# JMIsham/flink

Hardware: AMD Instinct MI355X
Metric: records/sec keyed windowed aggregation at 1/2/4/8 GPUs; % of HBM roofline (higher is better)
Workload: dtype int64

## Files before the change

flink_amd/csrc/fw_device.hip:

```cpp
#include <hip/hip_runtime.h>
#include <hip/hip_ext.h>

#include <algorithm>
#include <rocprim/device/device_radix_sort.hpp>

#include "../../include/flink_window.h"
#include "fw_internal.h"

namespace {

constexpr int64_t LMAX = INT64_MAX;
constexpr int64_t LMIN = INT64_MIN;
typedef long long i64x2 __attribute__((ext_vector_type(2)));
typedef uint32_t u32x4 __attribute__((ext_vector_type(4)));

#include "fw_jmath.h"
__device__ __forceinline__ uint64_t fmix64_inv(uint64_t x) {
  x ^= x >> 33;
  x *= 0x9cb4b2f8129337dbull;
  x ^= x >> 33;
  x *= 0x4f74430c22a54005ull;
  x ^= x >> 33;
  return x;
}
// ... 334 lines not shown
    }
  }
  return -1;
}
template <bool OWN = false>
__device__ __forceinline__ int32_t region_claim(const Region& r, uint64_t h, uint32_t word) {
  for (uint32_t i = 0; i <= r.mask; i++) {
    const uint32_t s = ((uint32_t)h + i) & r.mask;
    if ((OWN ? ld_state_wg(r.state + s) : ld_state(r.state + s)) != SLOT_EMPTY) continue;
    if ((OWN ? cas_state_wg(r.state + s, SLOT_EMPTY, word) : atomicCAS(r.state + s, SLOT_EMPTY, word)) == SLOT_EMPTY)
      return (int32_t)s;
  }
  return -1;
}


constexpr uint32_t TAINT_BUSY = 0x80000000u;
constexpr int TAINT_MAX_PROBES = 64;
__device__ __forceinline__ bool taint_insert(const DevCfg& c, int64_t key) {
  uint32_t s = taint_slot0(c, key);
  for (int probes = 0; probes < TAINT_MAX_PROBES;) {
    const uint32_t cur = __hip_atomic_load(&c.taint_state[s], __ATOMIC_RELAXED, __HIP_MEMORY_SCOPE_AGENT);
    __atomic_signal_fence(__ATOMIC_ACQUIRE);
    if (cur == c.taint_epoch) {
      if (__hip_atomic_load(&c.taint_key[s], __ATOMIC_RELAXED, __HIP_MEMORY_SCOPE_AGENT) == (uint64_t)key) return true;
      s = (s + 1) & c.taint_mask;
      probes++;
      continue;
    }
    if (cur == (c.taint_epoch | TAINT_BUSY)) continue;
    if (atomicCAS(&c.taint_state[s], cur, c.taint_epoch | TAINT_BUSY) == cur) {
      __hip_atomic_store(&c.taint_key[s], (uint64_t)key, __ATOMIC_RELAXED, __HIP_MEMORY_SCOPE_AGENT);
      asm volatile("s_waitcnt vmcnt(0)" ::: "memory");
      __hip_atomic_store(&c.taint_state[s], c.taint_epoch, __ATOMIC_RELAXED, __HIP_MEMORY_SCOPE_AGENT);
      return true;
    }
  }
  return false;
}
__global__ __launch_bounds__(256) void k_taint(DevCfg c, int64_t wm, const int64_t* __restrict__ key,
                                               const int64_t* __restrict__ ts, int64_t n, Status* st) {
  int any = 0;
  for (int64_t i = (int64_t)blockIdx.x * blockDim.x + threadIdx.x; i < n; i += (int64_t)gridDim.x * blockDim.x) {
    if (!session_ordered(c, wm, ts[i])) continue;
    any = max(any, taint_insert(c, key[i]) ? 1 : 2);
  }
  if (any) atomicMax(&st->taint_any, any);
}

__device__ __forceinline__ int64_t rec_index(int64_t b, int j, int e) {
  return b + 2 * ((int64_t)j * blockDim.x + threadIdx.x) + e;
}
template <int NP, bool VAL>
__device__ __forceinline__ void load_records(const DevCfg& c, const int64_t* __restrict__ key, const int64_t* __restrict__ ts,
                                             const int64_t* __restrict__ val, const int32_t* __restrict__ kh, int64_t b,
                                             int64_t end, int64_t (&k)[2 * NP], int64_t (&t)[2 * NP], int64_t (&v)[2 * NP],
                                             int32_t (&h)[2 * NP]) {
  const bool hashed = c.key_kind == FW_KEY_HASHED;
#pragma unroll
  for (int j = 0; j < NP; j++) {
    const int64_t i = rec_index(b, j, 0);
    if (c.vec_in && i + 1 < end) {
      const i64x2 kk = *reinterpret_cast<const i64x2*>(key + i);
      const i64x2 tt = *reinterpret_cast<const i64x2*>(ts + i);
      k[2 * j] = kk.x, k[2 * j + 1] = kk.y;
      t[2 * j] = tt.x, t[2 * j + 1] = tt.y;
      if (VAL) {
        const i64x2 vv = *reinterpret_cast<const i64x2*>(val + i);
        v[2 * j] = vv.x, v[2 * j + 1] = vv.y;
      }
      if (hashed) {
        const int2 hh = *reinterpret_cast<const int2*>(kh + i);
        h[2 * j] = hh.x, h[2 * j + 1] = hh.y;
      }
    } else {
#pragma unroll
      for (int e = 0; e < 2; e++) {
        const bool in = i + e < end;
        k[2 * j + e] = in ? key[i + e] : 0;
        t[2 * j + e] = in ? ts[i + e] : 0;
        if (VAL) v[2 * j + e] = in ? val[i + e] : 0;
        if (hashed) h[2 * j + e] = in ? kh[i + e] : 0;
      }
    }
  }
}
__device__ __forceinline__ int32_t tile_of_block(int32_t T) {
  const int32_t b = blockIdx.x;
  if (!FW_XCD_TILES) return b;
  const int32_t per = T >> 3, rem = T & 7, g = b & 7;
  return g * per + min(g, rem) + (b >> 3);
}

enum { M_GEN = 0, M_TUMB = 1, M_PANE = 2 };
template <int MODE>
__device__ __forceinline__ void specialize(DevCfg& c) {
  if constexpr (MODE == M_TUMB) {
    c.assigner = FW_TUMBLING;
    c.panes = 0;
    c.wpr = 1;
    c.key_kind = FW_KEY_LONG;
  } else if constexpr (MODE == M_PANE) {
    c.assigner = FW_SLIDING;
    c.panes = 1;
    c.key_kind = FW_KEY_LONG;
  }
}
__host__ __forceinline__ int stream_mode(const DevCfg& c) {
  if (c.key_kind != FW_KEY_LONG) return M_GEN;
  if (c.assigner == FW_TUMBLING) return M_TUMB;
  return c.panes ? M_PANE : M_GEN;
}

enum { RSV_OVER = 0, RSV_KG = 1, RSV_TS = 2, RSV_LATE = 4 };

template <int MODE>
__global__ __launch_bounds__(FW_TILE_THREADS) void k_classify_hist(DevCfg c, int64_t wm, const int64_t* __restrict__ key,
                                                                   const int64_t* __restrict__ ts,
                                                                   const int32_t* __restrict__ kh, int64_t n, int32_t T,
                                                                   uint32_t* __restrict__ hist, Status* st,
                                                                   const uint32_t* __restrict__ rsv) {
  specialize<MODE>(c);
  if (rsv && !rsv[c.P + RSV_OVER]) {
    if (blockIdx.x == 0 && threadIdx.x == 0) {
      if (rsv[c.P + RSV_KG]) atomicAdd(&st->kg_errors, (int)rsv[c.P + RSV_KG]);
      if (rsv[c.P + RSV_TS]) atomicAdd(&st->ts_errors, (int)rsv[c.P + RSV_TS]);
      const unsigned long long late = *reinterpret_cast<const unsigned long long*>(rsv + c.P + RSV_LATE);
      if (late) atomicAdd(&st->late_dropped, late);
    }
    return;
  }
  if (rsv && blockIdx.x == 0 && threadIdx.x == 0) {
    if (rsv[c.P + FW_RSV_NARROW])
      atomicAdd(&st->narrow_misses, 1);
    else
      atomicAdd(&st->rsv_fallbacks, 1);
  }
  extern __shared__ uint32_t lh[];
  for (int i = threadIdx.x; i <= c.P; i += blockDim.x) lh[i] = 0;
  __syncthreads();
  const int32_t tile = blockIdx.x;
  const int64_t base = (int64_t)tile * FW_TILE;
  const int64_t end = min(n, base + (int64_t)FW_TILE);
  int bad_kg = 0, bad_ts = 0, wide = 0;
  unsigned slow = 0;
  const int taint = c.assigner == FW_SESSION ? st->taint_any : 0;
  for (int64_t b = base; b < end; b += (int64_t)blockDim.x * FW_RPT) {
    int64_t k[FW_RPT], t[FW_RPT], v[FW_RPT];
    int32_t h[FW_RPT];
    load_records<FW_RPT / 2, false>(c, key, ts, nullptr, kh, b, end, k, t, v, h);
#pragma unroll
    for (int j = 0; j < FW_RPT; j++) {
      const int64_t i = rec_index(b, j >> 1, j & 1);
      if (i >= end) continue;
      const int32_t p = partition_of(c, k[j], c.key_kind == FW_KEY_HASHED ? h[j] : key_hash_of(c.key_kind, k[j], kh, i));
      if (p < 0) {
        bad_kg++;
        continue;
      }
      int64_t last = 0;
      int nw = 0;
      const int cls = classify(c, wm, t[j], &last, &nw, k[j], taint);
      if (cls == CLS_NORMAL) {
        atomicAdd(&lh[p], 1u);
        if (c.compact && compact_delta(c, last) < 0) wide = 1;
      } else if (cls == CLS_SLOW)
        slow++;
      else if (cls == CLS_BADTS)
        bad_ts++;
    }
  }
  if (slow) atomicAdd(&lh[c.P], slow);
  __syncthreads();
  for (int i = threadIdx.x; i <= c.P; i += blockDim.x) hist[(int64_t)i * T + tile] = lh[i];
  if (threadIdx.x == 0) hist[(int64_t)(c.P + 1) * T + tile] = lh[c.P];
  if (bad_kg) atomicAdd(&st->kg_errors, bad_kg);
  if (bad_ts) atomicAdd(&st->ts_errors, bad_ts);
  if (wide) atomicOr(c.wide, 1);
}

constexpr int SCAN_T = 1024, SCAN_E = 4, SCAN_B = SCAN_T * SCAN_E;

__device__ __forceinline__ uint32_t block_excl_scan(uint32_t v, uint32_t* sw, uint32_t* total) {
  const int lane = __lane_id(), wid = threadIdx.x >> 6;
  uint32_t x = v;
#pragma unroll
  for (int o = 1; o < 64; o <<= 1) {
    uint32_t y = __shfl_up(x, o, 64);
    if (lane >= o) x += y;
  }
  if (lane == 63) sw[wid] = x;
  __syncthreads();
  if (threadIdx.x == 0) {
    uint32_t run = 0;
    const int nw = blockDim.x >> 6;
    for (int w = 0; w < nw; w++) {
      uint32_t t = sw[w];
      sw[w] = run;
      run += t;
    }
    sw[nw] = run;
  }
  __syncthreads();
  *total = sw[blockDim.x >> 6];
  uint32_t r = sw[wid] + x - v;
  __syncthreads();
  return r;
}

__global__ __launch_bounds__(SCAN_T) void k_scan_blocks(uint32_t* data, int64_t m, uint32_t* sums, const uint32_t* gate) {
  if (gate && !*gate) return;
  __shared__ uint32_t sw[SCAN_T / 64 + 1];
  const int64_t base = (int64_t)blockIdx.x * SCAN_B + (int64_t)threadIdx.x * SCAN_E;
  uint32_t v[SCAN_E];
  uint32_t local = 0;
#pragma unroll
  for (int e = 0; e < SCAN_E; e++) {
    v[e] = base + e < m ? data[base + e] : 0u;
    local += v[e];
  }
  uint32_t total;
  uint32_t off = block_excl_scan(local, sw, &total);
#pragma unroll
  for (int e = 0; e < SCAN_E; e++) {
    if (base + e < m) data[base + e] = off;
    off += v[e];
  }
  if (threadIdx.x == 0) sums[blockIdx.x] = total;
}
__global__ __launch_bounds__(SCAN_T) void k_scan_top(uint32_t* sums, int64_t nb, const uint32_t* gate) {
  if (gate && !*gate) return;
  __shared__ uint32_t sw[SCAN_T / 64 + 1];
  uint32_t carry = 0;
  for (int64_t b0 = 0; b0 < nb; b0 += SCAN_T) {
    const int64_t i = b0 + threadIdx.x;
    uint32_t v = i < nb ? sums[i] : 0u, total;
    uint32_t off = block_excl_scan(v, sw, &total);
    if (i < nb) sums[i] = off + carry;
    carry += total;
  }
}
__global__ __launch_bounds__(SCAN_T) void k_scan_add(uint32_t* data, int64_t m, const uint32_t* sums, const uint32_t* gate) {
  if (gate && !*gate) return;
  const uint32_t add = sums[blockIdx.x];
  const int64_t base = (int64_t)blockIdx.x * SCAN_B;
  for (int e = threadIdx.x; e < SCAN_B; e += SCAN_T)
    if (base + e < m) data[base + e] += add;
}

__global__ __launch_bounds__(SCAN_T) void k_scan_gated(uint32_t* data, int64_t m, const uint32_t* gate) {
  if (!*gate) return;
  __shared__ uint32_t sw[SCAN_T / 64 + 1];
  uint32_t carry = 0;
  for (int64_t b0 = 0; b0 < m; b0 += SCAN_B) {
    const int64_t base = b0 + (int64_t)threadIdx.x * SCAN_E;
    uint32_t v[SCAN_E];
    uint32_t local = 0;
#pragma unroll
    for (int e = 0; e < SCAN_E; e++) {
      v[e] = base + e < m ? data[base + e] : 0u;
      local += v[e];
    }
    uint32_t total;
    uint32_t off = block_excl_scan(local, sw, &total) + carry;
#pragma unroll
    for (int e = 0; e < SCAN_E; e++) {
      if (base + e < m) data[base + e] = off;
      off += v[e];
    }
    carry += total;
    __syncthreads();
  }
}

__device__ __forceinline__ uint32_t dpp_swap1(uint32_t x) {
  return (uint32_t)__builtin_amdgcn_mov_dpp((int)x, 0xB1, 0xF, 0xF, false);
}
__device__ __forceinline__ int64_t dpp_swap1(int64_t x) {
  const uint32_t lo = dpp_swap1((uint32_t)(uint64_t)x), hi = dpp_swap1((uint32_t)((uint64_t)x >> 32));
  return (int64_t)(((uint64_t)hi << 32) | lo);
}
__device__ __forceinline__ void store_pair(PRec* part, bool valid, uint32_t pos, i64x2 a, i64x2 b) {
  const bool odd = __lane_id() & 1;
  const i64x2 send = odd ? a : b;
  const i64x2 recv = {dpp_swap1((int64_t)send.x), dpp_swap1((int64_t)send.y)};
  const uint32_t ppos = dpp_swap1(pos);
  const bool pval = dpp_swap1((uint32_t)valid) != 0;
  if (odd ? pval : valid) reinterpret_cast<i64x2*>(part + (odd ? ppos : pos))[odd] = odd ? recv : a;
  if (odd ? valid : pval) reinterpret_cast<i64x2*>(part + (odd ? pos : ppos))[odd] = odd ? b : recv;
}
// ... 7 lines not shown
  __syncthreads();
  const int64_t tbase = (int64_t)tile * FW_TILE;
  const int64_t tend = min(n, tbase + (int64_t)FW_TILE);
  unsigned long long late = 0;
  const int taint = c.assigner == FW_SESSION ? st->taint_any : 0;
  const bool cmp = c.compact && !*c.wide;
  for (int64_t b = tbase; b < tend; b += (int64_t)blockDim.x * FW_RPT) {
    int64_t k[FW_RPT], t[FW_RPT], v[FW_RPT];
    int32_t hh[FW_RPT];
    load_records<FW_RPT / 2, true>(c, key, ts, val, kh, b, tend, k, t, v, hh);
#pragma unroll
    for (int j = 0; j < FW_RPT; j++) {
      const int64_t i = rec_index(b, j >> 1, j & 1);
      bool norm = false;
      uint32_t pos = 0;
      int64_t last = 0;
      int nwin = 0;
      if (i < tend) {
        const int32_t h = c.key_kind == FW_KEY_HASHED ? hh[j] : key_hash_of(c.key_kind, k[j], kh, i);
        const int32_t p = partition_of(c, k[j], h);
        if (p >= 0) {
          const int cls = classify(c, wm, t[j], &last, &nwin, k[j], taint);
          if (cls == CLS_NORMAL) {
            pos = atomicAdd(&base[p], 1u);
            norm = true;
          } else if (cls == CLS_LATE) {
            if (c.side_output)
              side_one(side, st, k[j], t[j], v[j]);
            else
              late++;
          }
        }
      }
      if (c.diag & (DIAG_SCATTER_NO_STORE | DIAG_SCATTER_LINEAR | DIAG_SCATTER_SINGLE | DIAG_SCATTER_HALF |
                    DIAG_SCATTER_NT)) {
        if (c.diag & DIAG_SCATTER_NO_STORE) {
          asm volatile("" ::"v"(pos), "v"(k[j]), "v"(last), "v"(v[j]));
          continue;
        }
        if (c.diag & DIAG_SCATTER_LINEAR) pos = (uint32_t)i;
        if ((c.diag & DIAG_SCATTER_HALF) && norm) {
          i64x2* dst = reinterpret_cast<i64x2*>(part) + pos;
          if (c.diag & DIAG_SCATTER_NT)
            __builtin_nontemporal_store(i64x2{k[j] ^ last, v[j]}, dst);
          else
            *dst = i64x2{k[j] ^ last, v[j]};
          continue;
        }
        if ((c.diag & DIAG_SCATTER_NT) && norm) {
          i64x2* dst = reinterpret_cast<i64x2*>(part + pos);
          __builtin_nontemporal_store(i64x2{k[j], last}, dst);
          __builtin_nontemporal_store(i64x2{v[j], (long long)nwin}, dst + 1);
          continue;
        }
        if (norm) {
          i64x2* dst = reinterpret_cast<i64x2*>(part + pos);
          dst[0] = i64x2{k[j], last};
          dst[1] = i64x2{v[j], (long long)nwin};
        }
        continue;
      }
      if (cmp) {
        if (norm) reinterpret_cast<i64x2*>(part)[pos] = i64x2{compact_encode(c, k[j], compact_delta(c, last)), v[j]};
        continue;
      }
      const int64_t nwf = agg_ordinal(c) ? (i << 16) | nwin : (int64_t)nwin;
      store_pair(part, norm, pos, i64x2{k[j], last}, i64x2{v[j], (long long)nwf});
    }
  }
  if (late) atomicAdd(&st->late_dropped, late);
}
template <int MODE>
__global__ __launch_bounds__(FW_TILE_THREADS, FW_SCATTER_WAVES) void k_scatter(DevCfg c, int64_t wm, const int64_t* __restrict__ key,
                                                             const int64_t* __restrict__ ts,
                                                             const int64_t* __restrict__ val,
                                                             const int32_t* __restrict__ kh, int64_t n, int32_t T,
                                                             const uint32_t* __restrict__ offs, PRec* __restrict__ part,
                                                             DevSide side, Status* st) {
  specialize<MODE>(c);
  extern __shared__ uint32_t base[];
  scatter_direct(c, wm, key, ts, val, kh, n, T, offs, part, side, st, base, tile_of_block(T));
}

template <int MODE, int RR, bool RSV, bool NW = false>
__device__ __forceinline__ void scatter_staged_body(DevCfg c, int64_t wm, const int64_t* __restrict__ key,
                                                    const int64_t* __restrict__ ts, const int64_t* __restrict__ val,
                                                    const int32_t* __restrict__ kh, int64_t n, int32_t T,
                                                    const uint32_t* __restrict__ offs, PRec* __restrict__ part,
                                                    DevSide side, Status* st, uint32_t* rsv, int64_t rcap) {
  specialize<MODE>(c);
  extern __shared__ __attribute__((aligned(16))) uint8_t sraw[];
  i64x2* stg = reinterpret_cast<i64x2*>(sraw);
  uint64_t* stg8 = reinterpret_cast<uint64_t*>(sraw);
  uint16_t* sp = reinterpret_cast<uint16_t*>(sraw + (size_t)RR * (NW ? 8 : 16));
  uint32_t* gb = reinterpret_cast<uint32_t*>(sp + RR);
  uint32_t* cs = gb + c.P;
  uint32_t* wsum = cs + c.P + 1;
  const int32_t tile = tile_of_block(T);
  if constexpr (!RSV) {
    const bool cmp = c.compact && !*c.wide;
    if (!cmp) {
      scatter_direct(c, wm, key, ts, val, kh, n, T, offs, part, side, st, gb, tile);
      return;
    }
    for (int i = threadIdx.x; i < c.P; i += FW_TILE_THREADS) gb[i] = offs[(int64_t)i * T + tile];
  }
  const int64_t tbase = (int64_t)tile * FW_TILE;
  const int64_t tend = min(n, tbase + (int64_t)FW_TILE);
  unsigned long long late = 0;
  int bad_kg = 0, bad_ts = 0, over = 0, nmiss = 0;
  constexpr int RPT = RR / FW_TILE_THREADS;
  const int ppt = (c.P + FW_TILE_THREADS - 1) / FW_TILE_THREADS;
  i64x2* out = reinterpret_cast<i64x2*>(part);
  uint64_t* out8 = reinterpret_cast<uint64_t*>(part);
  for (int64_t b = tbase; b < tend; b += RR) {
    for (int i = threadIdx.x; i <= c.P; i += FW_TILE_THREADS) cs[i] = 0;
    __syncthreads();
    uint32_t rk[RPT];
    uint32_t pj[RPT];
    int64_t w[RPT], v[RPT];
#pragma unroll
    for (int hf = 0; hf < 2; hf++) {
      constexpr int H = RPT / 2;
      const int64_t bh = b + (int64_t)hf * H * FW_TILE_THREADS;
      int64_t k[H], t[H], vh[H];
      int32_t hh[H];
      load_records<H / 2, true>(c, key, ts, val, kh, bh, tend, k, t, vh, hh);
#pragma unroll
      for (int j = 0; j < H; j++) {
        const int jj = hf * H + j;
        const int64_t i = rec_index(bh, j >> 1, j & 1);
        pj[jj] = 0xffffffffu;
        v[jj] = vh[j];
        if (i >= tend) continue;
        const int32_t h = c.key_kind == FW_KEY_HASHED ? hh[j] : key_hash_of(c.key_kind, k[j], kh, i);
        const int32_t p = partition_of(c, k[j], h);
        if (p < 0) {
          bad_kg++;
          continue;
        }
        int64_t last = 0;
        int nwin = 0;
        const int cls = classify(c, wm, t[j], &last, &nwin, k[j], 0);
        if (cls == CLS_NORMAL) {
          const int64_t d = compact_delta(c, last);
          if (RSV && d < 0) {
            over = 1;
            continue;
          }
          if constexpr (NW) {
            uint64_t nw;
            if (!narrow_encode(c, k[j], d, vh[j], &nw)) {
              over = 1;
              nmiss = 1;
              continue;
            }
            w[jj] = (int64_t)nw;
          } else {
            w[jj] = compact_encode(c, k[j], d);
          }
          rk[jj] = atomicAdd(&cs[p], 1u);
          pj[jj] = (uint32_t)p;
        } else if (cls == CLS_LATE) {
          if (!RSV && c.side_output)
            side_one(side, st, k[j], t[j], vh[j]);
          else
            late++;
        } else if (cls == CLS_BADTS) {
          bad_ts++;
        }
      }
    }
    __syncthreads();
    constexpr int CQ = ((RSV ? FW_GMAX_P : FW_STAGED_MAX_P) + FW_TILE_THREADS - 1) / FW_TILE_THREADS;
    uint32_t cq[CQ], sum = 0;
#pragma unroll
    for (int q = 0; q < CQ; q++) {
      const int pp = threadIdx.x * ppt + q;
      cq[q] = q < ppt && pp < c.P ? cs[pp] : 0u;
      sum += cq[q];
    }
    uint32_t total;
    uint32_t e = block_excl_scan(sum, wsum, &total);
#pragma unroll
    for (int q = 0; q < CQ; q++) {
      const int pp = threadIdx.x * ppt + q;
      if (q < ppt && pp < c.P) cs[pp] = e;
      e += cq[q];
    }
    if (threadIdx.x == 0) cs[c.P] = total;
    __syncthreads();
#pragma unroll
    for (int j = 0; j < RPT; j++) {
      if (pj[j] == 0xffffffffu) continue;
      const uint32_t pos = cs[pj[j]] + rk[j];
      if constexpr (NW)
        stg8[pos] = (uint64_t)w[j];
      else
        stg[pos] = i64x2{w[j], v[j]};
      sp[pos] = (uint16_t)pj[j];
    }
    if constexpr (RSV) {
      for (int i = threadIdx.x; i < c.P; i += FW_TILE_THREADS) {
        const uint32_t m = cs[i + 1] - cs[i];
        if (m == 0) continue;
        const uint32_t g = atomicAdd(&rsv[i], m);
        if ((int64_t)g + m > rcap) {
          over = 1;
          gb[i] = 0xffffffffu;
        } else {
          gb[i] = (uint32_t)((int64_t)i * rcap + g);
        }
      }
    }
    __syncthreads();
    for (uint32_t i = threadIdx.x; i < total; i += FW_TILE_THREADS) {
      const uint32_t pp = sp[i];
      if (RSV && gb[pp] == 0xffffffffu) continue;
      if constexpr (NW)
        out8[gb[pp] + (i - cs[pp])] = stg8[i];
      else
        out[gb[pp] + (i - cs[pp])] = stg[i];
    }
    __syncthreads();
    if constexpr (!RSV) {
      for (int i = threadIdx.x; i < c.P; i += FW_TILE_THREADS) gb[i] += cs[i + 1] - cs[i];
      __syncthreads();
    }
  }
  if constexpr (RSV) {
    if (over) rsv[c.P + RSV_OVER] = 1;
    if (NW && nmiss) rsv[c.P + FW_RSV_NARROW] = 1;
    if (bad_kg) atomicAdd(&rsv[c.P + RSV_KG], (uint32_t)bad_kg);
    if (bad_ts) atomicAdd(&rsv[c.P + RSV_TS], (uint32_t)bad_ts);
    if (late) atomicAdd(reinterpret_cast<unsigned long long*>(rsv + c.P + RSV_LATE), late);
  } else if (late) {
    atomicAdd(&st->late_dropped, late);
  }
}
template <int MODE, int RR>
__global__ __launch_bounds__(FW_TILE_THREADS) void k_scatter_staged(DevCfg c, int64_t wm, const int64_t* __restrict__ key,
                                                                   const int64_t* __restrict__ ts,
                                                                   const int64_t* __restrict__ val,
                                                                   const int32_t* __restrict__ kh, int64_t n, int32_t T,
                                                                   const uint32_t* __restrict__ offs,
                                                                   PRec* __restrict__ part, DevSide side, Status* st,
                                                                   const uint32_t* __restrict__ gate) {
  if (gate && !gate[0]) return;
  scatter_staged_body<MODE, RR, false>(c, wm, key, ts, val, kh, n, T, offs, part, side, st, nullptr, 0);
}
template <int RR, bool NW>
__global__ __launch_bounds__(FW_TILE_THREADS) void k_scatter_rsv(DevCfg c, int64_t wm, const int64_t* __restrict__ key,
                                                                const int64_t* __restrict__ ts,
                                                                const int64_t* __restrict__ val,
                                                                const int32_t* __restrict__ kh, int64_t n, int32_t T,
                                                                PRec* __restrict__ part, uint32_t* rsv, int64_t rcap) {
  scatter_staged_body<M_TUMB, RR, true, NW>(c, wm, key, ts, val, kh, n, T, nullptr, part, DevSide{}, nullptr, rsv, rcap);
}

__global__ __launch_bounds__(FW_TILE_THREADS) void k_scatter_ordered(DevCfg c, int64_t wm, const int64_t* __restrict__ key,
                                                                     const int64_t* __restrict__ ts,
                                                                     const int64_t* __restrict__ val,
                                                                     const int32_t* __restrict__ kh, int64_t n,
                                                                     int32_t T, const uint32_t* __restrict__ srow,
                                                                     int64_t* __restrict__ sk, int64_t* __restrict__ stt,
                                                                     int64_t* __restrict__ sv, int32_t* __restrict__ skh, const Status* st) {
  const uint32_t* tile_slow = srow + T;
  if (tile_slow[blockIdx.x] == 0) return;
  const int taint = c.assigner == FW_SESSION ? st->taint_any : 0;
  __shared__ uint32_t wtot[FW_TILE_THREADS / 64];
  const uint32_t slow_base = srow[blockIdx.x] - srow[0];
  const int64_t tbase = (int64_t)blockIdx.x * FW_TILE;
  const int64_t tend = min(n, tbase + (int64_t)FW_TILE);
  const int lane = __lane_id(), wid = threadIdx.x >> 6, nw = blockDim.x >> 6;
  uint32_t running = 0;
  for (int64_t j = tbase; j < tend; j += blockDim.x) {
    const int64_t i = j + threadIdx.x;
    int cls = CLS_SKIP;
    int32_t p = -1, h = 0;
    int64_t k = 0, t = 0, v = 0;
    if (i < tend) {
      k = key[i];
      t = ts[i];
      v = val[i];
      h = key_hash_of(c.key_kind, k, kh, i);
      p = partition_of(c, k, h);
      if (p >= 0) {
        int64_t last = 0;
        int nw = 0;
        cls = classify(c, wm, t, &last, &nw, k, taint);
      }
    }
    const bool is_slow = cls == CLS_SLOW;
    const uint64_t ball = __ballot(is_slow);
    if (lane == 0) wtot[wid] = (uint32_t)__popcll(ball);
    __syncthreads();
    uint32_t woff = 0, tot = 0;
    for (int w = 0; w < nw; w++) {
      const uint32_t x = wtot[w];
      woff += w < wid ? x : 0u;
      tot += x;
    }
    if (is_slow) {
      const uint32_t pos = slow_base + running + woff + (uint32_t)__popcll(ball & lanemask_lt());
      sk[pos] = k;
      stt[pos] = t;
      sv[pos] = v;
      skh[pos] = h;
      if (agg_ordinal(c)) c.slow_ord[pos] = c.ord_base + i;
    }
    running += tot;
    __syncthreads();
  }
}

constexpr int LDS_BUCKETS = FW_LDS_SLOTS / 4;
struct AggLds {
  uint32_t tag[FW_LDS_SLOTS];
  uint32_t cnt[FW_LDS_SLOTS];
  i64x2 kv[FW_LDS_SLOTS];
  int64_t mn[FW_LDS_SLOTS];
  int64_t mx[FW_LDS_SLOTS];
  int64_t sum[FW_LDS_SLOTS];
  int32_t slot[FW_LDS_SLOTS];
  int fill;
  int anyfail;
  int spill;
  int last;
  int nnew;
  int live;
  unsigned long long flushed;
  int64_t min_timer;
  int hl_lo, hl_take, hl_idx;
  long long hl_bump;
  const int64_t* byv;
  int64_t byb;
};
enum : uint32_t { LT_EMPTY = 0, LT_BUSY = 1 };

__device__ __forceinline__ uint32_t lds_hash(int64_t key, int64_t start) {
// ... 6809 lines not shown
void launch_displaced_any(const DevCfg& c, const int64_t* ts, int64_t n, int32_t* flag, hipStream_t s) {
  const unsigned blocks = (unsigned)std::min<int64_t>(1024, (n + 255) / 256);
  hipLaunchKernelGGL(k_displaced_any, dim3(blocks), dim3(256), 0, s, c, ts, n, flag);
}
void launch_rsv_reset(uint32_t* rsv, int32_t words, const Status* st, hipStream_t s) {
  hipLaunchKernelGGL(k_rsv_reset, dim3((unsigned)std::min(64, (words + 255) / 256)), dim3(256), 0, s, rsv, words, st);
}
void launch_scan(uint32_t* data, int64_t m, uint32_t* scratch, hipStream_t s, const uint32_t* gate) {
  if (gate) {
    hipLaunchKernelGGL(k_scan_gated, dim3(1), dim3(SCAN_T), 0, s, data, m, gate);
    return;
  }
  const int64_t nb = (m + SCAN_B - 1) / SCAN_B;
  hipLaunchKernelGGL(k_scan_blocks, dim3((unsigned)nb), dim3(SCAN_T), 0, s, data, m, scratch, gate);
  hipLaunchKernelGGL(k_scan_top, dim3(1), dim3(SCAN_T), 0, s, scratch, nb, gate);
  hipLaunchKernelGGL(k_scan_add, dim3((unsigned)nb), dim3(SCAN_T), 0, s, data, m, (const uint32_t*)scratch, gate);
}

void launch_taint(const DevCfg& c, int64_t wm, const int64_t* key, const int64_t* ts, int64_t n, Status* st,
                  hipStream_t s) {
  const int64_t blocks = std::min<int64_t>((n + 255) / 256, 2048);
  if (blocks > 0) hipLaunchKernelGGL(k_taint, dim3((unsigned)blocks), dim3(256), 0, s, c, wm, key, ts, n, st);
}

void launch_scatter(const DevCfg& c, int64_t wm, const int64_t* key, const int64_t* ts, const int64_t* val,
                    const int32_t* kh, int64_t n, int32_t T, uint32_t* offs, PRec* part, int64_t* sk, int64_t* stt,
                    int64_t* sv, int32_t* skh, DevSide side, Status* st, hipStream_t s, const uint32_t* gate) {
  const size_t lds = (size_t)c.P * sizeof(uint32_t);
  const uint32_t* o = offs;
  static const bool no_staged = getenv("FW_NO_STAGED") && atoi(getenv("FW_NO_STAGED"));
  if (c.compact && c.P <= (gate ? FW_GMAX_P : FW_STAGED_MAX_P) && stream_mode(c) != M_GEN && (!no_staged || gate)) {
    const bool big = c.P <= 1024;
    const int rr = big ? 8192 : 4096;
    const size_t sl = (size_t)rr * (sizeof(i64x2) + sizeof(uint16_t)) + (2 * (size_t)c.P + 1) * sizeof(uint32_t) +
                      (FW_TILE_THREADS / 64 + 1) * sizeof(uint32_t);
    static bool attr = false;
    if (!attr) {
      (void)hipFuncSetAttribute((const void*)k_scatter_staged<M_TUMB, 8192>, hipFuncAttributeMaxDynamicSharedMemorySize, 160 * 1024);
      (void)hipFuncSetAttribute((const void*)k_scatter_staged<M_TUMB, 4096>, hipFuncAttributeMaxDynamicSharedMemorySize, 160 * 1024);
      (void)hipFuncSetAttribute((const void*)k_scatter_staged<M_PANE, 8192>, hipFuncAttributeMaxDynamicSharedMemorySize, 160 * 1024);
      (void)hipFuncSetAttribute((const void*)k_scatter_staged<M_PANE, 4096>, hipFuncAttributeMaxDynamicSharedMemorySize, 160 * 1024);
      attr = true;
    }
    const bool tumb = stream_mode(c) == M_TUMB;
    if (tumb && big)
      hipLaunchKernelGGL((k_scatter_staged<M_TUMB, 8192>), dim3(T), dim3(FW_TILE_THREADS), sl, s, c, wm, key, ts, val, kh, n,
                         T, o, part, side, st, gate);
    else if (tumb)
      hipLaunchKernelGGL((k_scatter_staged<M_TUMB, 4096>), dim3(T), dim3(FW_TILE_THREADS), sl, s, c, wm, key, ts, val, kh, n,
                         T, o, part, side, st, gate);
    else if (big)
      hipLaunchKernelGGL((k_scatter_staged<M_PANE, 8192>), dim3(T), dim3(FW_TILE_THREADS), sl, s, c, wm, key, ts, val, kh, n,
                         T, o, part, side, st, gate);
    else
      hipLaunchKernelGGL((k_scatter_staged<M_PANE, 4096>), dim3(T), dim3(FW_TILE_THREADS), sl, s, c, wm, key, ts, val, kh, n,
                         T, o, part, side, st, gate);
  } else
  switch (stream_mode(c)) {
    case M_TUMB:
      hipLaunchKernelGGL(k_scatter<M_TUMB>, dim3(T), dim3(FW_TILE_THREADS), lds, s, c, wm, key, ts, val, kh, n, T, o, part,
                         side, st);
      break;
    case M_PANE:
      hipLaunchKernelGGL(k_scatter<M_PANE>, dim3(T), dim3(FW_TILE_THREADS), lds, s, c, wm, key, ts, val, kh, n, T, o, part,
                         side, st);
      break;
    default:
      hipLaunchKernelGGL(k_scatter<M_GEN>, dim3(T), dim3(FW_TILE_THREADS), lds, s, c, wm, key, ts, val, kh, n, T, o, part,
                         side, st);
  }
  if (!c.dense)
    hipLaunchKernelGGL(k_scatter_ordered, dim3(T), dim3(FW_TILE_THREADS), 0, s, c, wm, key, ts, val, kh, n, T,
                       (const uint32_t*)(offs + (int64_t)c.P * T), sk, stt, sv, skh, (const Status*)st);
}

bool rsv_eligible(const DevCfg& c) {
  static const bool off = getenv("FW_NO_RSV") && atoi(getenv("FW_NO_RSV"));
  return !off && c.dense && c.compact && !c.side_output && c.P <= FW_GMAX_P && stream_mode(c) == M_TUMB;
}
void launch_scatter_rsv(const DevCfg& c, int64_t wm, const int64_t* key, const int64_t* ts, const int64_t* val,
                        const int32_t* kh, int64_t n, int32_t T, PRec* part, uint32_t* rsv, int64_t rcap, hipStream_t s) {
  const bool big = c.P <= 1024;
  const int rr = big ? 8192 : 4096;
  const size_t sl = (size_t)rr * ((c.narrow ? 8 : sizeof(i64x2)) + sizeof(uint16_t)) +
                    (2 * (size_t)c.P + 1) * sizeof(uint32_t) + (FW_TILE_THREADS / 64 + 1) * sizeof(uint32_t);
  static bool attr = false;
  if (!attr) {
    for (const void* f : {(const void*)k_scatter_rsv<8192, false>, (const void*)k_scatter_rsv<4096, false>,
                          (const void*)k_scatter_rsv<8192, true>, (const void*)k_scatter_rsv<4096, true>})
      (void)hipFuncSetAttribute(f, hipFuncAttributeMaxDynamicSharedMemorySize, 160 * 1024);
    attr = true;
  }
  if (c.narrow && big)
    FW_LAUNCH_MAIN((k_scatter_rsv<8192, true>), dim3(T), dim3(FW_TILE_THREADS), sl, s, c, wm, key, ts, val, kh, n, T,
                   part, rsv, 2 * rcap);
  else if (c.narrow)
    FW_LAUNCH_MAIN((k_scatter_rsv<4096, true>), dim3(T), dim3(FW_TILE_THREADS), sl, s, c, wm, key, ts, val, kh, n, T,
                   part, rsv, 2 * rcap);
  else if (big)
    FW_LAUNCH_MAIN((k_scatter_rsv<8192, false>), dim3(T), dim3(FW_TILE_THREADS), sl, s, c, wm, key, ts, val, kh, n, T,
                   part, rsv, rcap);
  else
    FW_LAUNCH_MAIN((k_scatter_rsv<4096, false>), dim3(T), dim3(FW_TILE_THREADS), sl, s, c, wm, key, ts, val, kh, n, T,
                   part, rsv, rcap);
}

int64_t pane_nt_floor(const DevCfg& c, int64_t wm) {
  if (!c.panes) return 0;
  const __int128 x = (__int128)wm - c.size + 2;
  __int128 r = ((__int128)c.offset - x) % c.slide;
  if (r < 0) r += c.slide;
  const __int128 e = x + r + c.size - 1;
  return e > (__int128)LMAX ? LMAX : e < (__int128)LMIN ? LMIN : (int64_t)e;
}

void launch_aggregate(const DevCfg& c0, int64_t wm, const PRec* part, const uint32_t* offs, int32_t T, DevTable tb,
                      AggProg prog, int resume, const AggHot* hot, int64_t n, Status* st, hipStream_t s,
                      const uint32_t* rsv, int64_t rcap, bool dn) {
  DevCfg c = c0;
  c.nt_floor = pane_nt_floor(c, wm);
  AggHot h{};
  unsigned grid = (unsigned)c.P;
  if (hot) {
    h = *hot;
    grid += (unsigned)((n + c.agg_chunk - 1) / c.agg_chunk);
    if (!resume) {
      hipLaunchKernelGGL(k_chunk_plan, dim3((c.P + 1 + 255) / 256), dim3(256), 0, s, c, offs, T, h);
      launch_scan(h.chunk_base, (int64_t)c.P + 1, h.scan_tmp, s);
    }
  }
  if (c.dense) {
    if (!resume && rsv && c.narrow && dn) {
      FW_LAUNCH_MAIN((k_dn_aggregate<1024, 4080, 2, 3, 8>), dim3(c.P), dim3(1024), 0, s, c, (const uint64_t*)part, tb,
                     prog, st, rsv, rcap);
    } else if (!resume && rsv && c.narrow && FW_DT_NDEPTH > 0)
      FW_LAUNCH_MAIN((k_dt_aggregate<DT_RECS, true, true>), dim3(c.P), dim3(FW_DT_THREADS), 0, s, c, (const void*)part, offs,
                     T, tb, prog, resume, st, rsv, rcap);
    else
      FW_LAUNCH_MAIN((k_dt_aggregate<DT_RECS, true>), dim3(c.P), dim3(FW_DT_THREADS), 0, s, c, (const void*)part, offs, T,
                     tb, prog, resume, st, rsv, rcap);
    if (resume)
      hipLaunchKernelGGL((k_dt_aggregate<DT_RECS, false>), dim3(c.P), dim3(FW_DT_THREADS), 0, s, c, (const void*)part,
                         offs, T, tb, prog, 1, st, rsv, rcap);
    return;
  }
  const dim3 b(FW_AGG_THREADS);
  const bool first = agg_ordinal(c), pool = c.pool_bytes != 0;
  if (c.assigner == FW_SESSION && first)
    hipLaunchKernelGGL((k_aggregate<FW_AGG_RPT, true, true, false>), dim3(grid), b, 0, s, c, wm, part, offs, T, tb, prog,
                       resume, st, h);
  else if (c.assigner == FW_SESSION && pool)
    hipLaunchKernelGGL((k_aggregate<FW_SESS_RPT, true, false, true>), dim3(grid), b, 0, s, c, wm, part, offs, T, tb, prog,
                       resume, st, h);
  else if (c.assigner == FW_SESSION)
    hipLaunchKernelGGL((k_aggregate<FW_SESS_RPT, true, false, false>), dim3(grid), b, 0, s, c, wm, part, offs, T, tb,
                       prog, resume, st, h);
  else if (first)
    hipLaunchKernelGGL((k_aggregate<FW_AGG_RPT, false, true, false>), dim3(grid), b, 0, s, c, wm, part, offs, T, tb,
                       prog, resume, st, h);
  else if (pool)
    hipLaunchKernelGGL((k_aggregate<FW_POOL_RPT, false, false, true>), dim3(grid), b, 0, s, c, wm, part, offs, T, tb,
                       prog, resume, st, h);
  else
    hipLaunchKernelGGL((k_aggregate<FW_PLAIN_RPT, false, false, false>), dim3(grid), b, 0, s, c, wm, part, offs, T, tb,
                       prog, resume, st, h);
}

void launch_hll_update(const DevCfg& c, const PRec* part, const uint32_t* offs, int32_t T, int64_t n, DevTable tb,
                       Status* st, hipStream_t s) {
  if (n <= 0) return;
  const dim3 grid((unsigned)((n + FW_HLL_CHUNK - 1) / FW_HLL_CHUNK));
  if (c.assigner == FW_SESSION)
    hipLaunchKernelGGL(k_hll_update_sessions, grid, dim3(256), 0, s, c, part, offs, T, tb, st);
  else if (c.assigner == FW_SLIDING)
    hipLaunchKernelGGL(k_hll_update<true>, grid, dim3(256), 0, s, c, part, offs, T, tb, st);
  else
    hipLaunchKernelGGL(k_hll_update<false>, grid, dim3(256), 0, s, c, part, offs, T, tb, st);
}

void launch_row_update(const DevCfg& c, const PRec* part, const uint32_t* offs, int32_t T, int64_t n, DevTable tb,
                       Status* st, hipStream_t s) {
  if (n <= 0) return;
  const dim3 grid((unsigned)((n + FW_HLL_CHUNK - 1) / FW_HLL_CHUNK));
  if (c.assigner == FW_SESSION)
    hipLaunchKernelGGL(k_row_update<2>, grid, dim3(256), 0, s, c, part, offs, T, tb, st);
  else if (c.assigner == FW_SLIDING)
    hipLaunchKernelGGL(k_row_update<1>, grid, dim3(256), 0, s, c, part, offs, T, tb, st);
// ... 309 lines not shown
```

Baseline: 57.11 billion.

## Make reservation scatter persistent with software-pipelined loads and overlapped flush

Pulls the reservation-based scatter out of the shared staged body and turns it into a persistent kernel whose grid is capped at the compute-unit count. Each block walks rounds of records, prefetching the next round's key/ts (and value) columns while it classifies the current one. The previous round's staged LDS buffer is flushed to global memory in the same iteration, with double-buffered counters and a shuffle-based tile scan. This is meant to hide HBM load latency and cut per-tile launch and sync overhead, at the cost of more register pressure and more complex boundary handling.

```diff
diff --git a/flink_amd/csrc/fw_device.hip b/flink_amd/csrc/fw_device.hip
--- a/flink_amd/csrc/fw_device.hip
+++ b/flink_amd/csrc/fw_device.hip
@@ -440,6 +440,36 @@
         if (VAL) v[2 * j + e] = in ? val[i + e] : 0;
         if (hashed) h[2 * j + e] = in ? kh[i + e] : 0;
       }
+    }
+  }
+}
+__device__ __forceinline__ int64_t tile_rec_index(int64_t b, int j, int e) {
+  return b + 2 * ((int64_t)j * FW_TILE_THREADS + threadIdx.x) + e;
+}
+typedef i64x2 i64x2_a8 __attribute__((aligned(8)));
+template <int N>
+__device__ __forceinline__ int64_t pair_at(const int64_t (&a)[N], int j, int64_t i, int64_t n) {
+  return (j & 1) == 0 && i == n - 1 ? a[j + 1] : a[j];
+}
+template <int NP, int COLS>
+__device__ __forceinline__ void load_pairs(const int64_t* __restrict__ key, const int64_t* __restrict__ ts,
+                                           const int64_t* __restrict__ val, int64_t b, int64_t n, int64_t (&k)[2 * NP],
+                                           int64_t (&t)[2 * NP], int64_t (&v)[2 * NP]) {
+#pragma unroll
+  for (int j = 0; j < NP; j++) {
+    const int64_t i = tile_rec_index(b, j, 0);
+    const int64_t ia = min(i, n - 2);
+    if constexpr (COLS & 1) {
+      const i64x2 kk = *reinterpret_cast<const i64x2_a8*>(key + ia);
+      k[2 * j] = kk.x, k[2 * j + 1] = kk.y;
+    }
+    if constexpr (COLS & 2) {
+      const i64x2 tt = *reinterpret_cast<const i64x2_a8*>(ts + ia);
+      t[2 * j] = tt.x, t[2 * j + 1] = tt.y;
+    }
+    if constexpr (COLS & 4) {
+      const i64x2 vv = *reinterpret_cast<const i64x2_a8*>(val + ia);
+      v[2 * j] = vv.x, v[2 * j + 1] = vv.y;
     }
   }
 }
@@ -564,6 +594,28 @@
   uint32_t r = sw[wid] + x - v;
   __syncthreads();
   return r;
+}
+
+__device__ __forceinline__ uint32_t tile_excl_scan(uint32_t v, uint32_t* sw, uint32_t* total) {
+  constexpr int NWV = FW_TILE_THREADS / 64;
+  const int lane = __lane_id(), wid = threadIdx.x >> 6;
+  uint32_t x = v;
+#pragma unroll
+  for (int o = 1; o < 64; o <<= 1) {
+    uint32_t y = __shfl_up(x, o, 64);
+    if (lane >= o) x += y;
+  }
+  if (lane == 63) sw[wid] = x;
+  __syncthreads();
+  uint32_t y = lane < NWV ? sw[lane] : 0u;
+#pragma unroll
+  for (int o = 1; o < NWV; o <<= 1) {
+    uint32_t z = __shfl_up(y, o, 64);
+    if (lane >= o) y += z;
+  }
+  *total = __shfl(y, NWV - 1, 64);
+  const uint32_t before = __shfl(y, max(wid - 1, 0), 64);
+  return (wid ? before : 0u) + x - v;
 }
 
 __global__ __launch_bounds__(SCAN_T) void k_scan_blocks(uint32_t* data, int64_t m, uint32_t* sums, const uint32_t* gate) {
@@ -737,37 +789,32 @@
   scatter_direct(c, wm, key, ts, val, kh, n, T, offs, part, side, st, base, tile_of_block(T));
 }
 
-template <int MODE, int RR, bool RSV, bool NW = false>
+template <int MODE, int RR>
 __device__ __forceinline__ void scatter_staged_body(DevCfg c, int64_t wm, const int64_t* __restrict__ key,
                                                     const int64_t* __restrict__ ts, const int64_t* __restrict__ val,
                                                     const int32_t* __restrict__ kh, int64_t n, int32_t T,
                                                     const uint32_t* __restrict__ offs, PRec* __restrict__ part,
-                                                    DevSide side, Status* st, uint32_t* rsv, int64_t rcap) {
+                                                    DevSide side, Status* st) {
   specialize<MODE>(c);
   extern __shared__ __attribute__((aligned(16))) uint8_t sraw[];
   i64x2* stg = reinterpret_cast<i64x2*>(sraw);
-  uint64_t* stg8 = reinterpret_cast<uint64_t*>(sraw);
-  uint16_t* sp = reinterpret_cast<uint16_t*>(sraw + (size_t)RR * (NW ? 8 : 16));
+  uint16_t* sp = reinterpret_cast<uint16_t*>(sraw + (size_t)RR * 16);
   uint32_t* gb = reinterpret_cast<uint32_t*>(sp + RR);
   uint32_t* cs = gb + c.P;
   uint32_t* wsum = cs + c.P + 1;
   const int32_t tile = tile_of_block(T);
-  if constexpr (!RSV) {
-    const bool cmp = c.compact && !*c.wide;
-    if (!cmp) {
-      scatter_direct(c, wm, key, ts, val, kh, n, T, offs, part, side, st, gb, tile);
-      return;
-    }
-    for (int i = threadIdx.x; i < c.P; i += FW_TILE_THREADS) gb[i] = offs[(int64_t)i * T + tile];
-  }
+  const bool cmp = c.compact && !*c.wide;
+  if (!cmp) {
+    scatter_direct(c, wm, key, ts, val, kh, n, T, offs, part, side, st, gb, tile);
+    return;
+  }
+  for (int i = threadIdx.x; i < c.P; i += FW_TILE_THREADS) gb[i] = offs[(int64_t)i * T + tile];
   const int64_t tbase = (int64_t)tile * FW_TILE;
   const int64_t tend = min(n, tbase + (int64_t)FW_TILE);
   unsigned long long late = 0;
-  int bad_kg = 0, bad_ts = 0, over = 0, nmiss = 0;
   constexpr int RPT = RR / FW_TILE_THREADS;
   const int ppt = (c.P + FW_TILE_THREADS - 1) / FW_TILE_THREADS;
   i64x2* out = reinterpret_cast<i64x2*>(part);
-  uint64_t* out8 = reinterpret_cast<uint64_t*>(part);
   for (int64_t b = tbase; b < tend; b += RR) {
     for (int i = threadIdx.x; i <= c.P; i += FW_TILE_THREADS) cs[i] = 0;
     __syncthreads();
@@ -790,44 +837,24 @@
         if (i >= tend) continue;
         const int32_t h = c.key_kind == FW_KEY_HASHED ? hh[j] : key_hash_of(c.key_kind, k[j], kh, i);
         const int32_t p = partition_of(c, k[j], h);
-        if (p < 0) {
-          bad_kg++;
-          continue;
-        }
+        if (p < 0) continue;
         int64_t last = 0;
         int nwin = 0;
         const int cls = classify(c, wm, t[j], &last, &nwin, k[j], 0);
         if (cls == CLS_NORMAL) {
-          const int64_t d = compact_delta(c, last);
-          if (RSV && d < 0) {
-            over = 1;
-            continue;
-          }
-          if constexpr (NW) {
-            uint64_t nw;
-            if (!narrow_encode(c, k[j], d, vh[j], &nw)) {
-              over = 1;
-              nmiss = 1;
-              continue;
-            }
-            w[jj] = (int64_t)nw;
-          } else {
-            w[jj] = compact_encode(c, k[j], d);
-          }
+          w[jj] = compact_encode(c, k[j], compact_delta(c, last));
           rk[jj] = atomicAdd(&cs[p], 1u);
           pj[jj] = (uint32_t)p;
         } else if (cls == CLS_LATE) {
-          if (!RSV && c.side_output)
+          if (c.side_output)
             side_one(side, st, k[j], t[j], vh[j]);
           else
             late++;
-        } else if (cls == CLS_BADTS) {
-          bad_ts++;
         }
       }
     }
     __syncthreads();
-    constexpr int CQ = ((RSV ? FW_GMAX_P : FW_STAGED_MAX_P) + FW_TILE_THREADS - 1) / FW_TILE_THREADS;
+    constexpr int CQ = (FW_STAGED_MAX_P + FW_TILE_THREADS - 1) / FW_TILE_THREADS;
     uint32_t cq[CQ], sum = 0;
 #pragma unroll
     for (int q = 0; q < CQ; q++) {
@@ -849,49 +876,19 @@
     for (int j = 0; j < RPT; j++) {
       if (pj[j] == 0xffffffffu) continue;
       const uint32_t pos = cs[pj[j]] + rk[j];
-      if constexpr (NW)
-        stg8[pos] = (uint64_t)w[j];
-      else
-        stg[pos] = i64x2{w[j], v[j]};
+      stg[pos] = i64x2{w[j], v[j]};
       sp[pos] = (uint16_t)pj[j];
-    }
-    if constexpr (RSV) {
-      for (int i = threadIdx.x; i < c.P; i += FW_TILE_THREADS) {
-        const uint32_t m = cs[i + 1] - cs[i];
-        if (m == 0) continue;
-        const uint32_t g = atomicAdd(&rsv[i], m);
-        if ((int64_t)g + m > rcap) {
-          over = 1;
-          gb[i] = 0xffffffffu;
-        } else {
-          gb[i] = (uint32_t)((int64_t)i * rcap + g);
-        }
-      }
     }
     __syncthreads();
     for (uint32_t i = threadIdx.x; i < total; i += FW_TILE_THREADS) {
       const uint32_t pp = sp[i];
-      if (RSV && gb[pp] == 0xffffffffu) continue;
-      if constexpr (NW)
-        out8[gb[pp] + (i - cs[pp])] = stg8[i];
-      else
-        out[gb[pp] + (i - cs[pp])] = stg[i];
+      out[gb[pp] + (i - cs[pp])] = stg[i];
     }
     __syncthreads();
-    if constexpr (!RSV) {
-      for (int i = threadIdx.x; i < c.P; i += FW_TILE_THREADS) gb[i] += cs[i + 1] - cs[i];
-      __syncthreads();
-    }
-  }
-  if constexpr (RSV) {
-    if (over) rsv[c.P + RSV_OVER] = 1;
-    if (NW && nmiss) rsv[c.P + FW_RSV_NARROW] = 1;
-    if (bad_kg) atomicAdd(&rsv[c.P + RSV_KG], (uint32_t)bad_kg);
-    if (bad_ts) atomicAdd(&rsv[c.P + RSV_TS], (uint32_t)bad_ts);
-    if (late) atomicAdd(reinterpret_cast<unsigned long long*>(rsv + c.P + RSV_LATE), late);
-  } else if (late) {
-    atomicAdd(&st->late_dropped, late);
-  }
+    for (int i = threadIdx.x; i < c.P; i += FW_TILE_THREADS) gb[i] += cs[i + 1] - cs[i];
+    __syncthreads();
+  }
+  if (late) atomicAdd(&st->late_dropped, late);
 }
 template <int MODE, int RR>
 __global__ __launch_bounds__(FW_TILE_THREADS) void k_scatter_staged(DevCfg c, int64_t wm, const int64_t* __restrict__ key,
@@ -902,15 +899,190 @@
                                                                    PRec* __restrict__ part, DevSide side, Status* st,
                                                                    const uint32_t* __restrict__ gate) {
   if (gate && !gate[0]) return;
-  scatter_staged_body<MODE, RR, false>(c, wm, key, ts, val, kh, n, T, offs, part, side, st, nullptr, 0);
+  scatter_staged_body<MODE, RR>(c, wm, key, ts, val, kh, n, T, offs, part, side, st);
+}
+
+struct RsvCounts {
+  unsigned long long late = 0;
+  int bad_kg = 0, bad_ts = 0, over = 0, nmiss = 0;
+};
+template <bool NW>
+__device__ __forceinline__ int32_t rsv_record(const DevCfg& c, int64_t wm, int64_t k, int64_t t, int64_t v,
+                                              const int32_t* __restrict__ kh, int64_t i, int64_t* w, RsvCounts& n) {
+  const int32_t p = partition_of(c, k, key_hash_of(c.key_kind, k, kh, i));
+  if (p < 0) {
+    n.bad_kg++;
+    return -1;
+  }
+  int64_t last = 0;
+  int nwin = 0;
+  const int cls = classify(c, wm, t, &last, &nwin, k, 0);
+  if (cls == CLS_NORMAL) {
+    const int64_t d = compact_delta(c, last);
+    if (d < 0) {
+      n.over = 1;
+      return -1;
+    }
+    if constexpr (NW) {
+      uint64_t nw;
+      if (!narrow_encode(c, k, d, v, &nw)) {
+        n.over = 1;
+        n.nmiss = 1;
+        return -1;
+      }
+      *w = (int64_t)nw;
+    } else {
+      *w = compact_encode(c, k, d);
+    }
+    return p;
+  }
+  if (cls == CLS_LATE)
+    n.late++;
+  else if (cls == CLS_BADTS)
+    n.bad_ts++;
+  return -1;
+}
+template <bool NW>
+__device__ __forceinline__ void rsv_counts_out(const DevCfg& c, uint32_t* rsv, const RsvCounts& n) {
+  if (n.over) rsv[c.P + RSV_OVER] = 1;
+  if (NW && n.nmiss) rsv[c.P + FW_RSV_NARROW] = 1;
+  if (n.bad_kg) atomicAdd(&rsv[c.P + RSV_KG], (uint32_t)n.bad_kg);
+  if (n.bad_ts) atomicAdd(&rsv[c.P + RSV_TS], (uint32_t)n.bad_ts);
+  if (n.late) atomicAdd(reinterpret_cast<unsigned long long*>(rsv + c.P + RSV_LATE), n.late);
 }
 template <int RR, bool NW>
 __global__ __launch_bounds__(FW_TILE_THREADS) void k_scatter_rsv(DevCfg c, int64_t wm, const int64_t* __restrict__ key,
                                                                 const int64_t* __restrict__ ts,
                                                                 const int64_t* __restrict__ val,
-                                                                const int32_t* __restrict__ kh, int64_t n, int32_t T,
+                                                                const int32_t* __restrict__ kh, int64_t n,
                                                                 PRec* __restrict__ part, uint32_t* rsv, int64_t rcap) {
-  scatter_staged_body<M_TUMB, RR, true, NW>(c, wm, key, ts, val, kh, n, T, nullptr, part, DevSide{}, nullptr, rsv, rcap);
+  static_assert(FW_TILE % RR == 0 && RR % (4 * FW_TILE_THREADS) == 0 && RR <= 65536 && FW_GMAX_P < 65535);
+  specialize<M_TUMB>(c);
+  i64x2* out = reinterpret_cast<i64x2*>(part);
+  uint64_t* out8 = reinterpret_cast<uint64_t*>(part);
+  RsvCounts cnt;
+  if (n < 2) {
+    if (n == 1 && blockIdx.x == 0 && threadIdx.x == 0) {
+      int64_t w = 0;
+      const int64_t v0 = val[0];
+      const int32_t p = rsv_record<NW>(c, wm, key[0], ts[0], v0, kh, 0, &w, cnt);
+      if (p >= 0) {
+        const uint32_t g = atomicAdd(&rsv[p], 1u);
+        if ((int64_t)g + 1 > rcap)
+          cnt.over = 1;
+        else if constexpr (NW)
+          out8[(int64_t)p * rcap + g] = (uint64_t)w;
+        else
+          out[(int64_t)p * rcap + g] = i64x2{w, v0};
+      }
+      rsv_counts_out<NW>(c, rsv, cnt);
+    }
+    return;
+  }
+  extern __shared__ __attribute__((aligned(16))) uint8_t sraw[];
+  i64x2* stg = reinterpret_cast<i64x2*>(sraw);
+  uint64_t* stg8 = reinterpret_cast<uint64_t*>(sraw);
+  uint16_t* sp = reinterpret_cast<uint16_t*>(sraw + (size_t)RR * (NW ? 8 : 16));
+  uint32_t* gb = reinterpret_cast<uint32_t*>(sp + RR);
+  uint32_t* cs = gb + c.P;
+  uint32_t* cp = cs + c.P;
+  uint32_t* wsum = gb + 3 * c.P;
+  constexpr int RPT = RR / FW_TILE_THREADS;
+  constexpr int H = RPT / 2;
+  constexpr int PPT = RR == 8192 ? 1 : 2;
+  int64_t r = blockIdx.x;
+  int64_t b = min(r * RR, n), end = min(n, b + RR);
+  int64_t k[2][H], t[2][H], v[2][H];
+#pragma unroll
+  for (int hf = 0; hf < 2; hf++) load_pairs<H / 2, NW ? 7 : 3>(key, ts, val, b + hf * (RR / 2), n, k[hf], t[hf], v[hf]);
+  for (int i = threadIdx.x; i < c.P; i += FW_TILE_THREADS) cs[i] = 0;
+  uint32_t staged = 0;
+  uint32_t gm[PPT] = {}, gg[PPT];
+  __syncthreads();
+  for (;;) {
+    const bool more = b < n;
+    const int64_t bn = min((r += gridDim.x) * RR, n), endn = min(n, bn + RR);
+    uint32_t pr[RPT];
+    int64_t w[RPT];
+#pragma unroll
+    for (int hf = 0; hf < 2; hf++) {
+#pragma unroll
+      for (int jh = 0; jh < H; jh++) {
+        const int j = hf * H + jh;
+        const int64_t i = tile_rec_index(b + hf * (RR / 2), jh >> 1, jh & 1);
+        pr[j] = 0xffffffffu;
+        if (i >= end) continue;
+        const int32_t p = rsv_record<NW>(c, wm, pair_at(k[hf], jh, i, n), pair_at(t[hf], jh, i, n),
+                                         NW ? pair_at(v[hf], jh, i, n) : 0, kh, i, &w[j], cnt);
+        if (p >= 0) pr[j] = (uint32_t)p << 16 | atomicAdd(&cs[p], 1u);
+      }
+      if constexpr (NW) load_pairs<H / 2, 7>(key, ts, val, bn + hf * (RR / 2), n, k[hf], t[hf], v[hf]);
+    }
+    if constexpr (!NW) {
+#pragma unroll
+      for (int hf = 0; hf < 2; hf++) {
+        load_pairs<H / 2, 3>(key, ts, val, bn + hf * (RR / 2), n, k[hf], t[hf], v[hf]);
+        load_pairs<H / 2, 4>(key, ts, val, b + hf * (RR / 2), n, k[hf], t[hf], v[hf]);
+      }
+    }
+#pragma unroll
+    for (int q = 0; q < PPT; q++) {
+      const int i = threadIdx.x + q * FW_TILE_THREADS;
+      if (gm[q] == 0) continue;
+      if ((int64_t)gg[q] + gm[q] > rcap) {
+        cnt.over = 1;
+        gb[i] = 0xffffffffu;
+      } else {
+        gb[i] = (uint32_t)((int64_t)i * rcap + gg[q]);
+      }
+    }
+    __syncthreads();
+    for (uint32_t i = threadIdx.x; i < staged; i += FW_TILE_THREADS) {
+      const uint32_t pp = sp[i];
+      if (gb[pp] == 0xffffffffu) continue;
+      if constexpr (NW)
+        out8[gb[pp] + (i - cp[pp])] = stg8[i];
+      else
+        out[gb[pp] + (i - cp[pp])] = stg[i];
+    }
+    if (!more) break;
+#pragma unroll
+    for (int q = 0; q < PPT; q++) {
+      const int i = threadIdx.x + q * FW_TILE_THREADS;
+      gm[q] = i < c.P ? cs[i] : 0u;
+      if (gm[q]) gg[q] = atomicAdd(&rsv[i], gm[q]);
+    }
+    uint32_t cq[PPT], sum = 0;
+#pragma unroll
+    for (int q = 0; q < PPT; q++) {
+      const int pp = threadIdx.x * PPT + q;
+      cq[q] = pp < c.P ? cs[pp] : 0u;
+      sum += cq[q];
+    }
+    uint32_t e = tile_excl_scan(sum, wsum, &staged);
+#pragma unroll
+    for (int q = 0; q < PPT; q++) {
+      const int pp = threadIdx.x * PPT + q;
+      if (pp < c.P) cs[pp] = e;
+      e += cq[q];
+    }
+    for (int i = threadIdx.x; i < c.P; i += FW_TILE_THREADS) cp[i] = 0;
+    __syncthreads();
+#pragma unroll
+    for (int j = 0; j < RPT; j++) {
+      if (pr[j] == 0xffffffffu) continue;
+      const uint32_t pos = cs[pr[j] >> 16] + (pr[j] & 0xffffu);
+      if constexpr (NW)
+        stg8[pos] = (uint64_t)w[j];
+      else
+        stg[pos] = i64x2{w[j], pair_at(v[j / H], j % H, tile_rec_index(b + (j / H) * (RR / 2), (j % H) >> 1, 0), n)};
+      sp[pos] = (uint16_t)(pr[j] >> 16);
+    }
+    b = bn, end = endn;
+    uint32_t* const x = cs;
+    cs = cp, cp = x;
+  }
+  rsv_counts_out<NW>(c, rsv, cnt);
 }
 
 __global__ __launch_bounds__(FW_TILE_THREADS) void k_scatter_ordered(DevCfg c, int64_t wm, const int64_t* __restrict__ key,
@@ -7886,8 +8058,8 @@
                         const int32_t* kh, int64_t n, int32_t T, PRec* part, uint32_t* rsv, int64_t rcap, hipStream_t s) {
   const bool big = c.P <= 1024;
   const int rr = big ? 8192 : 4096;
-  const size_t sl = (size_t)rr * ((c.narrow ? 8 : sizeof(i64x2)) + sizeof(uint16_t)) +
-                    (2 * (size_t)c.P + 1) * sizeof(uint32_t) + (FW_TILE_THREADS / 64 + 1) * sizeof(uint32_t);
+  const size_t sl = (size_t)rr * ((c.narrow ? 8 : sizeof(i64x2)) + sizeof(uint16_t)) + 3 * (size_t)c.P * sizeof(uint32_t) +
+                    (FW_TILE_THREADS / 64) * sizeof(uint32_t);
   static bool attr = false;
   if (!attr) {
     for (const void* f : {(const void*)k_scatter_rsv<8192, false>, (const void*)k_scatter_rsv<4096, false>,
@@ -7895,18 +8067,28 @@
       (void)hipFuncSetAttribute(f, hipFuncAttributeMaxDynamicSharedMemorySize, 160 * 1024);
     attr = true;
   }
+  static thread_local int cu_dev = -1, cus = 0;
+  int dev = 0;
+  (void)hipGetDevice(&dev);
+  if (dev != cu_dev) {
+    if (hipDeviceGetAttribute(&cus, hipDeviceAttributeMultiprocessorCount, dev) != hipSuccess || cus <= 0) cus = 256;
+    cu_dev = dev;
+  }
+  const int64_t rounds = (n + rr - 1) / rr;
+  const dim3 grid((unsigned)std::max<int64_t>(1, std::min<int64_t>(rounds, cus)));
+  (void)T;
   if (c.narrow && big)
-    FW_LAUNCH_MAIN((k_scatter_rsv<8192, true>), dim3(T), dim3(FW_TILE_THREADS), sl, s, c, wm, key, ts, val, kh, n, T,
-                   part, rsv, 2 * rcap);
+    FW_LAUNCH_MAIN((k_scatter_rsv<8192, true>), grid, dim3(FW_TILE_THREADS), sl, s, c, wm, key, ts, val, kh, n, part, rsv,
+                   2 * rcap);
   else if (c.narrow)
-    FW_LAUNCH_MAIN((k_scatter_rsv<4096, true>), dim3(T), dim3(FW_TILE_THREADS), sl, s, c, wm, key, ts, val, kh, n, T,
-                   part, rsv, 2 * rcap);
+    FW_LAUNCH_MAIN((k_scatter_rsv<4096, true>), grid, dim3(FW_TILE_THREADS), sl, s, c, wm, key, ts, val, kh, n, part, rsv,
+                   2 * rcap);
   else if (big)
-    FW_LAUNCH_MAIN((k_scatter_rsv<8192, false>), dim3(T), dim3(FW_TILE_THREADS), sl, s, c, wm, key, ts, val, kh, n, T,
-                   part, rsv, rcap);
+    FW_LAUNCH_MAIN((k_scatter_rsv<8192, false>), grid, dim3(FW_TILE_THREADS), sl, s, c, wm, key, ts, val, kh, n, part, rsv,
+                   rcap);
   else
-    FW_LAUNCH_MAIN((k_scatter_rsv<4096, false>), dim3(T), dim3(FW_TILE_THREADS), sl, s, c, wm, key, ts, val, kh, n, T,
-                   part, rsv, rcap);
+    FW_LAUNCH_MAIN((k_scatter_rsv<4096, false>), grid, dim3(FW_TILE_THREADS), sl, s, c, wm, key, ts, val, kh, n, part, rsv,
+                   rcap);
 }
 
 int64_t pane_nt_floor(const DevCfg& c, int64_t wm) {
```

Measured after the change: 61.71 billion, median of 6. 8.1% higher.
